# hao1635/FoundDiff

Measured on AMD Instinct MI355X. Metric: denoised CT slices/sec (512x512, 50 DDIM steps), higher is better.
Workload: dtype bf16; last 1 step(s): resolution levels 0-1 on the fp32s engine (fp32 storage, split-bf16 contractions: 3 bf16 MFMAs per product); 1 GPU; BASELINE configs[2]: 512x512 slice, 50-step DDIM, full FoundDiff UNet (dim 64, mults 1-2-4-8) + DA-CLIP RN50 cond, bf16; concurrent_sub_batches=2

## Files before the change

### founddiff_amd/csrc/fd_initconv.hip

```cpp
#include "fd_common.h"

namespace {

constexpr int IT = 16, IHY = IT + 6, IHX = IT + 8;

template <int NG>
__global__ __launch_bounds__(256, 2) void initconv7_kernel(const float *__restrict__ p0, const float *__restrict__ p1,
                                                          const float *__restrict__ p2, const bf16 *__restrict__ wk,
                                                          const float *__restrict__ bias, bf16 *__restrict__ out,
                                                          int H, int W) {
    __shared__ __attribute__((aligned(16))) uint2 sx[IHY * IHX];
    const int tid = threadIdx.x, lane = tid & 63, wave = tid >> 6;
    const int fr = lane & 15, fg = lane >> 4;
    const int tiles_x = W / IT;
    const int ty0 = (blockIdx.x / tiles_x) * IT, tx0 = (blockIdx.x % tiles_x) * IT;
    const int64_t img = blockIdx.y, plane = (int64_t)H * W;
    const int rperm = 8 * (fr >> 2) + (fr & 3);
    bf16x8 wa[NG][7], wb[NG][7];
#pragma unroll
    for (int g = 0; g < NG; ++g)
#pragma unroll
        for (int kh = 0; kh < 7; ++kh) {
            wa[g][kh] = *(const bf16x8 *)(wk + (int64_t)(32 * g + rperm) * 224 + kh * 32 + fg * 8);
            wb[g][kh] = *(const bf16x8 *)(wk + (int64_t)(32 * g + rperm + 4) * 224 + kh * 32 + fg * 8);
        }
    for (int i = tid; i < IHY * IHX; i += 256) {
        const int hy = i / IHX, hx = i - hy * IHX;
        const int y = ty0 + hy - 3, x = tx0 + hx - 3;
        float v0 = 0.f, v1 = 0.f, v2 = 0.f;
        if (y >= 0 && y < H && x >= 0 && x < W) {
            const int64_t o = img * plane + (int64_t)y * W + x;
            v0 = p0[o];
            if (p1) v1 = p1[o];
            if (p2) v2 = p2[o];
        }
        const bf16 b0 = (bf16)v0, b1 = (bf16)v1;
        uint2 wv;
        wv.x = (uint32_t)__builtin_bit_cast(uint16_t, b0) | ((uint32_t)__builtin_bit_cast(uint16_t, b1) << 16);
        if (p2) {
            const bf16 b2 = (bf16)v2;
            wv.y = (uint32_t)__builtin_bit_cast(uint16_t, b2);
        } else {
            const bf16 l0 = (bf16)(v0 - (float)b0), l1 = (bf16)(v1 - (float)b1);
            wv.y = (uint32_t)__builtin_bit_cast(uint16_t, l0) | ((uint32_t)__builtin_bit_cast(uint16_t, l1) << 16);
        }
        sx[i] = wv;
    }
    __syncthreads();
    float bs[NG][8];
#pragma unroll
    for (int g = 0; g < NG; ++g) {
        if (bias) load8(bias + 32 * g + 8 * fg, bs[g]);
        else {
#pragma unroll
            for (int e = 0; e < 8; ++e) bs[g][e] = 0.f;
        }
    }
    constexpr int CO = 32 * NG;
#pragma unroll 1
    for (int i = 0; i < 4; ++i) {
        const int ty = 4 * wave + i;
        f32x4 a0[NG], a1[NG];
#pragma unroll
        for (int g = 0; g < NG; ++g) { a0[g] = (f32x4){0.f, 0.f, 0.f, 0.f}; a1[g] = (f32x4){0.f, 0.f, 0.f, 0.f}; }
#pragma unroll
        for (int kh = 0; kh < 7; ++kh) {
            const uint2 *src = sx + (ty + kh) * IHX + fr + 2 * fg;
            const uint2 q0 = src[0], q1 = src[1];
            const u32x4 xv = {q0.x, q0.y, q1.x, q1.y};
            const bf16x8 xb = __builtin_bit_cast(bf16x8, xv);
#pragma unroll
            for (int g = 0; g < NG; ++g) {
                a0[g] = FD_MFMA16(wa[g][kh], xb, a0[g], 0, 0, 0);
                a1[g] = FD_MFMA16(wb[g][kh], xb, a1[g], 0, 0, 0);
            }
        }
        const int y = ty0 + ty, x = tx0 + fr;
        bf16 *op = out + ((img * H + y) * W + x) * CO + 8 * fg;
#pragma unroll
        for (int g = 0; g < NG; ++g) {
            float val[8];
#pragma unroll
            for (int e = 0; e < 4; ++e) { val[e] = a0[g][e] + bs[g][e]; val[4 + e] = a1[g][e] + bs[g][4 + e]; }
            store8(op + 32 * g, val);
        }
    }
}

template <int NG>
__global__ __launch_bounds__(256, 2) void initconv7_f32s_kernel(const float *__restrict__ p0, const float *__restrict__ p1,
                                                               const bf16 *__restrict__ wk, const bf16 *__restrict__ wl,
                                                               const float *__restrict__ bias, float *__restrict__ out,
                                                               int H, int W) {
    __shared__ __attribute__((aligned(16))) uint2 sx[IHY * IHX];
    const int tid = threadIdx.x, lane = tid & 63, wave = tid >> 6;
    const int fr = lane & 15, fg = lane >> 4;
    const int tiles_x = W / IT;
    const int ty0 = (blockIdx.x / tiles_x) * IT, tx0 = (blockIdx.x % tiles_x) * IT;
    const int64_t img = blockIdx.y, plane = (int64_t)H * W;
    const int rperm = 8 * (fr >> 2) + (fr & 3);
    for (int i = tid; i < IHY * IHX; i += 256) {
        const int hy = i / IHX, hx = i - hy * IHX;
        const int y = ty0 + hy - 3, x = tx0 + hx - 3;
        float v0 = 0.f, v1 = 0.f;
        if (y >= 0 && y < H && x >= 0 && x < W) {
            const int64_t o = img * plane + (int64_t)y * W + x;
            v0 = p0[o];
            v1 = p1[o];
        }
        const bf16 b0 = (bf16)v0, b1 = (bf16)v1;
        const bf16 l0 = (bf16)(v0 - (float)b0), l1 = (bf16)(v1 - (float)b1);
        uint2 wv;
        wv.x = (uint32_t)__builtin_bit_cast(uint16_t, b0) | ((uint32_t)__builtin_bit_cast(uint16_t, b1) << 16);
        wv.y = (uint32_t)__builtin_bit_cast(uint16_t, l0) | ((uint32_t)__builtin_bit_cast(uint16_t, l1) << 16);
        sx[i] = wv;
    }
    __syncthreads();
    constexpr int CO = 32 * NG;
#pragma unroll 1
    for (int g = 0; g < NG; ++g) {
        bf16x8 wa[7], wb[7], la[7], lb[7];
#pragma unroll
        for (int kh = 0; kh < 7; ++kh) {
            const int64_t oa = (int64_t)(32 * g + rperm) * 224 + kh * 32 + fg * 8, ob = oa + 4 * 224;
            wa[kh] = *(const bf16x8 *)(wk + oa);
            wb[kh] = *(const bf16x8 *)(wk + ob);
            la[kh] = *(const bf16x8 *)(wl + oa);
            lb[kh] = *(const bf16x8 *)(wl + ob);
        }
        float bs[8];
        if (bias) load8(bias + 32 * g + 8 * fg, bs);
        else {
#pragma unroll
            for (int e = 0; e < 8; ++e) bs[e] = 0.f;
        }
#pragma unroll 1
        for (int i = 0; i < 4; ++i) {
            const int ty = 4 * wave + i;
            f32x4 a0 = {0.f, 0.f, 0.f, 0.f}, a1 = {0.f, 0.f, 0.f, 0.f};
#pragma unroll
            for (int kh = 0; kh < 7; ++kh) {
                const uint2 *src = sx + (ty + kh) * IHX + fr + 2 * fg;
                const uint2 q0 = src[0], q1 = src[1];
                const u32x4 xv = {q0.x, q0.y, q1.x, q1.y};
                const bf16x8 xb = __builtin_bit_cast(bf16x8, xv);
                a0 = FD_MFMA16(la[kh], xb, a0, 0, 0, 0);
                a1 = FD_MFMA16(lb[kh], xb, a1, 0, 0, 0);
                a0 = FD_MFMA16(wa[kh], xb, a0, 0, 0, 0);
                a1 = FD_MFMA16(wb[kh], xb, a1, 0, 0, 0);
            }
            const int y = ty0 + ty, x = tx0 + fr;
            float *op = out + ((img * H + y) * W + x) * CO + 32 * g + 8 * fg;
            float val[8];
#pragma unroll
            for (int e = 0; e < 4; ++e) { val[e] = a0[e] + bs[e]; val[4 + e] = a1[e] + bs[4 + e]; }
            store8(op, val);
        }
    }
}

}

extern "C" int fd_init_conv7_f32s(const float *p0, const float *p1, const void *w_hi_packed, const void *w_lo_packed,
                                  const float *bias, void *out, int B, int H, int W, int Cout, void *stream) {
    FD_REQUIRE((Cout == 32 || Cout == 64) && H % IT == 0 && W % IT == 0, "fd_init_conv7_f32s: needs Cout in {32, 64}, H, W multiples "
               "of 16 (Cout=%d H=%d W=%d)", Cout, H, W);
    FD_REQUIRE(p0 && p1 && w_hi_packed && w_lo_packed && out, "fd_init_conv7_f32s: null pointer");
    FD_REQUIRE((((uintptr_t)bias | (uintptr_t)out | (uintptr_t)w_hi_packed | (uintptr_t)w_lo_packed) & 15) == 0, "fd_init_conv7_f32s: 16-byte alignment");
    dim3 grid((H / IT) * (W / IT), B), block(256);
    if (Cout == 64)
        hipLaunchKernelGGL(initconv7_f32s_kernel<2>, grid, block, 0, (hipStream_t)stream, p0, p1, (const bf16 *)w_hi_packed,
                           (const bf16 *)w_lo_packed, bias, (float *)out, H, W);
    else
        hipLaunchKernelGGL(initconv7_f32s_kernel<1>, grid, block, 0, (hipStream_t)stream, p0, p1, (const bf16 *)w_hi_packed,
                           (const bf16 *)w_lo_packed, bias, (float *)out, H, W);
    FD_LAUNCH_OK("fd_init_conv7_f32s");
    return FD_OK;
}

extern "C" int fd_init_conv7_ok(int dtype, int Cout, int H, int W) {
    return dtype == FD_BF16 && (Cout == 32 || Cout == 64) && H % IT == 0 && W % IT == 0;
}

extern "C" int fd_init_conv7(int dtype, const float *p0, const float *p1, const float *p2, const void *w_packed,
                             const float *bias, void *out, int B, int H, int W, int Cout, void *stream) {
    FD_REQUIRE(fd_init_conv7_ok(dtype, Cout, H, W), "fd_init_conv7: needs bf16, Cout in {32, 64}, H, W multiples of 16 "
               "(Cout=%d H=%d W=%d)", Cout, H, W);
    FD_REQUIRE(p0 && w_packed && out, "fd_init_conv7: null pointer");
    FD_REQUIRE(!bias || ((uintptr_t)bias & 15) == 0, "fd_init_conv7: bias must be 16-byte aligned");
    dim3 grid((H / IT) * (W / IT), B), block(256);
    if (Cout == 64)
        hipLaunchKernelGGL(initconv7_kernel<2>, grid, block, 0, (hipStream_t)stream, p0, p1, p2, (const bf16 *)w_packed, bias,
                           (bf16 *)out, H, W);
    else
        hipLaunchKernelGGL(initconv7_kernel<1>, grid, block, 0, (hipStream_t)stream, p0, p1, p2, (const bf16 *)w_packed, bias,
                           (bf16 *)out, H, W);
    FD_LAUNCH_OK("fd_init_conv7");
    return FD_OK;
}
```

### founddiff_amd/csrc/fd_scan.hip

```cpp
#include "fd_common.h"
#include <stdlib.h>

namespace {

struct ScanGeom {
    int B, H, W, D, N, R, CD;
    int H2, W2, L, CL, nch;
    const void *xw;
    float *xdbl_out;
    bool low_latency;
};

__device__ __forceinline__ void scan_pos(const ScanGeom &g, int k, int l, int &lrow, int &pix) {
    int h2, w2;
    if (k & 1) { w2 = l / g.H2; h2 = l - w2 * g.H2; }
    else { h2 = l / g.W2; w2 = l - h2 * g.W2; }
    lrow = h2 * g.W2 + w2;
    pix = (2 * h2 + (k & 1)) * g.W + 2 * w2 + (k >> 1);
}

template <typename T, int N, int R, bool FINAL, bool ODD, int CPL = 1>
__global__ __launch_bounds__(256, (N >= 32 ? 3 : (N >= 16 && R >= 16 ? 4 : (N >= 8 ? (CPL == 2 ? 4 : 5) : 1)))) void scan_chunk_kernel(const T *__restrict__ xc, const float *__restrict__ xdbl,
                                                        const float *__restrict__ dtw, const float *__restrict__ dtb,
                                                        const float *__restrict__ A, const float *__restrict__ Ds,
// ... 141 lines not shown
                    }
                }
            }
        }
    }
    if (FINAL || !g.xw)
    for (int idx = threadIdx.x; idx < (l1 - l0) * CD; idx += blockDim.x) {
        const int row = idx / CD, e = idx - row * CD;
        const int l = l0 + row;
        int h2, w2;
        if (odd) { w2 = l / g.H2; h2 = l - w2 * g.H2; }
        else { h2 = l / g.W2; w2 = l - h2 * g.W2; }
        float v = xb[(int64_t)(h2 * g.W2 + w2) * CD + e];
        if (LOG2U && FINAL && e >= R + N) v *= 0.6931471805599453f;
        sx[row * CDP + e] = v;
    }

    constexpr int NP = CPL == 2 ? N : N / 2, RP = CPL == 2 ? R : R / 2;
    f32x2 w[RP], a2[NP], h[NP];
    f32x2 bias2 = {0.f, 0.f}, Dd2 = {0.f, 0.f};
    float bias = 0.f, Dd = 0.f;
    const int64_t cbase = (((int64_t)bk * g.nch + chunk) * N) * g.D + d;
    if constexpr (CPL == 2) {
#pragma unroll
        for (int r = 0; r < R; ++r) w[r] = f32x2{dtw[(int64_t)kd * R + r], dtw[(int64_t)(kd + 1) * R + r]} * WS;
#pragma unroll
        for (int n = 0; n < N; ++n) a2[n] = f32x2{A[(int64_t)kd * N + n], A[(int64_t)(kd + 1) * N + n]} * AS;
        bias2 = f32x2{dtb[kd], dtb[kd + 1]} * WS;
        if (FINAL) Dd2 = f32x2{Ds[kd], Ds[kd + 1]};
#pragma unroll
        for (int n = 0; n < N; ++n) h[n] = FINAL ? *(const f32x2 *)&wsH[cbase + (int64_t)n * g.D] : f32x2{0.f, 0.f};
    } else {
#pragma unroll
        for (int r = 0; r < R / 2; ++r) w[r] = f32x2{dtw[(int64_t)kd * R + 2 * r], dtw[(int64_t)kd * R + 2 * r + 1]} * WS;
#pragma unroll
        for (int n = 0; n < N / 2; ++n)
            a2[n] = f32x2{A[(int64_t)kd * N + 2 * n], A[(int64_t)kd * N + 2 * n + 1]} * AS;
        bias = dtb[kd] * WS;
        Dd = FINAL ? Ds[kd] : 0.f;
        if (FINAL) {
#pragma unroll
            for (int n = 0; n < N / 2; ++n)
                h[n] = f32x2{wsH[cbase + (int64_t)(2 * n) * g.D], wsH[cbase + (int64_t)(2 * n + 1) * g.D]};
        } else {
#pragma unroll
            for (int n = 0; n < N / 2; ++n) h[n] = f32x2{0.f, 0.f};
        }
    }
    float sdt = 0.f;
    f32x2 sdt2 = {0.f, 0.f};
    const T *ub = xc + (int64_t)b * g.H * g.W * g.D;
    T *yb = FINAL ? y + (int64_t)b * g.H * g.W * g.D : nullptr;
    const int rowb = g.D * (int)sizeof(T);
    const int img_bytes = g.H * g.W * rowb;
    const __amdgpu_buffer_rsrc_t rs_u = __builtin_amdgcn_make_buffer_rsrc((void *)ub, 0, img_bytes, 0x00020000);
    const __amdgpu_buffer_rsrc_t rs_y = __builtin_amdgcn_make_buffer_rsrc((void *)(FINAL ? yb : (T *)ub), 0, img_bytes, 0x00020000);
    const int voff = d * (int)sizeof(T);
    auto ld_u = [&](int soff_) -> uint32_t {
        const int soff = __builtin_amdgcn_readfirstlane(soff_);
        if (ODD && soff < 0) return 0u;
        if constexpr (CPL == 2) return __builtin_amdgcn_raw_buffer_load_b32(rs_u, voff, soff, 0);
        else if constexpr (sizeof(T) == 2) return (uint32_t)__builtin_amdgcn_raw_buffer_load_b16(rs_u, voff, soff, 0);
        else return __builtin_amdgcn_raw_buffer_load_b32(rs_u, voff, soff, 0);
    };
    auto cvt_u = [&](uint32_t r) -> float {
        if constexpr (sizeof(T) == 2) return fd_h_lo(r);
        else return __builtin_bit_cast(float, r);
    };
    auto st_y = [&](int soff_, float v) {
        const int soff = __builtin_amdgcn_readfirstlane(soff_);
        if (ODD && soff < 0) return;
        if constexpr (sizeof(T) == 2) {
            const bf16 hv = fd_cvt_h(v);
            __builtin_amdgcn_raw_buffer_store_b16(__builtin_bit_cast(unsigned short, hv), rs_y, voff, soff, 0);
        } else {
            __builtin_amdgcn_raw_buffer_store_b32(__builtin_bit_cast(uint32_t, v), rs_y, voff, soff, 0);
        }
    };
    auto st_y2 = [&](int soff_, f32x2 v) {
        const int soff = __builtin_amdgcn_readfirstlane(soff_);
        if (ODD && soff < 0) return;
        typedef __attribute__((ext_vector_type(2))) bf16 bfx2;
        const bfx2 hv = {fd_cvt_h(v.x), fd_cvt_h(v.y)};
        __builtin_amdgcn_raw_buffer_store_b32(__builtin_bit_cast(uint32_t, hv), rs_y, voff, soff, 0);
    };
    const int NI = odd ? g.H2 : g.W2;
    const int s_i = odd ? 2 * g.W : 2, s_o = odd ? 2 : 2 * g.W;
    int ci = __builtin_amdgcn_readfirstlane(l0 % NI);
    int pixc = __builtin_amdgcn_readfirstlane(ph * g.W + pw + (l0 % NI) * s_i + (l0 / NI) * s_o);
    const int wrap_fix = s_o - NI * s_i;
    const int NO = odd ? g.W2 : g.H2;
    const bool padF = ODD && (odd ? ((g.H & 1) && ph) : ((g.W & 1) && pw));
    const bool padS = ODD && (odd ? ((g.W & 1) && pw) : ((g.H & 1) && ph));
    int co = __builtin_amdgcn_readfirstlane(l0 / NI);
    __syncthreads();

    constexpr int NXV = CPL == 2 ? ((FINAL ? CD : R + N) + 3) / 4 : 1;
    struct RowV { f32x4 v[NXV]; };
    auto ld_row = [&](int li) -> RowV {
        RowV q;
#pragma unroll
        for (int c = 0; c < NXV; ++c) q.v[c] = *(const f32x4 *)&sx[li * CDP + 4 * c];
        return q;
    };
    auto step = [&](const float *xr_lds, const RowV &rq, uint32_t uraw, int soff) {
        if constexpr (CPL == 2) {
            const auto xr = [&](int i) -> float { return rq.v[i >> 2][i & 3]; };
            const f32x2 u2 = {fd_h_lo(uraw), fd_h_hi(uraw)};
            f32x2 dv2 = bias2;
#pragma unroll
            for (int r = 0; r < R; ++r) dv2 = w[r] * xr(r) + dv2;
            f32x2 dt2;
            dt2.x = __builtin_amdgcn_logf(1.0f + __builtin_amdgcn_exp2f(fminf(dv2.x, 126.f)));
            dt2.y = __builtin_amdgcn_logf(1.0f + __builtin_amdgcn_exp2f(fminf(dv2.y, 126.f)));
            const f32x2 dtu2 = dt2 * u2;
            if (!FINAL) sdt2 += dt2;
            f32x2 acc2 = Dd2 * u2;
#pragma unroll
            for (int n = 0; n < N; ++n) {
                const f32x2 t = a2[n] * dt2;
                const f32x2 da = {__builtin_amdgcn_exp2f(t.x), __builtin_amdgcn_exp2f(t.y)};
                h[n] = da * h[n] + dtu2 * xr(R + n);
                if (FINAL) acc2 = h[n] * xr(R + N + n) + acc2;
            }
            if (FINAL) st_y2(soff, acc2);
        } else {
        const float u = cvt_u(uraw);
        const f32x2 *xr2 = (const f32x2 *)xr_lds;
        f32x2 dv2 = {bias, 0.f};
#pragma unroll
        for (int r = 0; r < R / 2; ++r) dv2 = w[r] * xr2[r] + dv2;
        const float dv = dv2.x + dv2.y;
        float dt;
        if constexpr (LOG2U) dt = __builtin_amdgcn_logf(1.0f + __builtin_amdgcn_exp2f(fminf(dv, 126.f)));
        else dt = fd_softplus_fast(dv);
        const float dtu = dt * u;
        if (!FINAL) sdt += dt;
        f32x2 acc2 = {0.f, 0.f};
#pragma unroll
        for (int n = 0; n < N / 2; ++n) {
            const f32x2 t = a2[n] * dt;
            const f32x2 da = {__builtin_amdgcn_exp2f(t.x), __builtin_amdgcn_exp2f(t.y)};
            h[n] = da * h[n] + xr2[R / 2 + n] * dtu;
            if (FINAL) acc2 = h[n] * xr2[R / 2 + N / 2 + n] + acc2;
        }
        if (FINAL) st_y(soff, acc2.x + acc2.y + Dd * u);
        }
    };
    auto advance = [&](int &soff) {
        soff = pixc * rowb;
        if (ODD && ((padF && ci == NI - 1) || (padS && co == NO - 1))) soff = -1;
        ++ci;
        const bool wrap = ci == NI;
        ci = wrap ? 0 : ci;
        if (ODD) co += wrap ? 1 : 0;
        pixc += s_i + (wrap ? wrap_fix : 0);
    };
    if constexpr (!FINAL && CPL == 2) {
        if (g.xw) {
            unsigned char *su = (unsigned char *)(sx + g.CL * CDP);
            const bf16 *Wk = (const bf16 *)g.xw + (int64_t)k * CD * g.D;
            const bf16 *ubx = (const bf16 *)xc + (int64_t)b * g.H * g.W * g.D;
            float *xo = g.xdbl_out + ((int64_t)k * g.B + b) * g.L * g.CD;
            constexpr int MB = (CD + 15) / 16, KSM = 4;
            const int fr = lane & 15, fg = lane >> 4;
            const int nblk = (l1 - l0 + 15) >> 4;
            struct BlkPos { int l, lrow; };
            auto bfetch = [&](int nb, BlkPos &q, bf16x8 (&bq)[KSM]) {
                const int l = l0 + nb * 16 + fr;
                int h2, w2;
                if (odd) { w2 = l / g.H2; h2 = l - w2 * g.H2; }
                else { h2 = l / g.W2; w2 = l - h2 * g.W2; }
                const int hh = 2 * h2 + ph, ww = 2 * w2 + pw;
                const bool inimg = l < l1 && hh < g.H && ww < g.W;
                const bf16 *px = ubx + ((int64_t)hh * g.W + ww) * g.D + 8 * fg;
                q.l = l;
                q.lrow = h2 * g.W2 + w2;
#pragma unroll
                for (int ks = 0; ks < KSM; ++ks) {
                    bq[ks] = (bf16x8){0, 0, 0, 0, 0, 0, 0, 0};
                    if (inimg) bq[ks] = *(const bf16x8 *)(px + 32 * ks);
                }
            };
            bf16x8 afr[MB][KSM];
#pragma unroll
            for (int mb = 0; mb < MB; ++mb) {
                const int e = mb * 16 + fr;
#pragma unroll
                for (int ks = 0; ks < KSM; ++ks) {
                    afr[mb][ks] = (bf16x8){0, 0, 0, 0, 0, 0, 0, 0};
                    if (e < CD) afr[mb][ks] = *(const bf16x8 *)(Wk + (int64_t)e * g.D + 32 * ks + 8 * fg);
                }
            }
            const int su_rd = ((lane >> 2) << 4) | ((lane & 3) << 2);
            auto ld_su = [&](int s_) -> uint32_t { return *(const uint32_t *)(su + s_ * 256 + (su_rd ^ ((s_ & 15) << 4))); };
            BlkPos cur, nxt;
            bf16x8 bcur[KSM], bnxt[KSM];
            bfetch(0, cur, bcur);
            for (int nb = 0; nb < nblk; ++nb) {
                const bool more = nb + 1 < nblk;
                if (more) bfetch(nb + 1, nxt, bnxt);
#pragma unroll
                for (int mb = 0; mb < MB; ++mb) {
                    f32x4 acc = {0.f, 0.f, 0.f, 0.f};
#pragma unroll
                    for (int ks = 0; ks < KSM; ++ks) acc = FD_MFMA16(afr[mb][ks], bcur[ks], acc, 0, 0, 0);
                    const int e0 = mb * 16 + 4 * fg;
                    if (cur.l < l1 && e0 < CD) {
                        *(f32x4 *)&sx[(nb * 16 + fr) * CDP + e0] = acc;
                        *(f32x4 *)&xo[(int64_t)cur.lrow * CD + e0] = acc;
                    }
                }
#pragma unroll
                for (int ks = 0; ks < KSM; ++ks) *(bf16x8 *)(su + fr * 256 + (((ks * 4 + fg) ^ fr) << 4)) = bcur[ks];
                const int ns = min(16, l1 - l0 - nb * 16);
                if (ns == 16) {
                    RowV r0 = ld_row(nb * 16);
                    uint32_t u0 = ld_su(0);
#pragma unroll
                    for (int st = 0; st < 16; ++st) {
                        RowV r1 = r0;
                        uint32_t u1 = u0;
                        if (st + 1 < 16) { r1 = ld_row(nb * 16 + st + 1); u1 = ld_su(st + 1); }
                        __builtin_amdgcn_sched_barrier(0);
                        step(nullptr, r0, u0, 0);
                        r0 = r1;
                        u0 = u1;
                    }
                } else {
                    for (int st = 0; st < ns; ++st) step(nullptr, ld_row(nb * 16 + st), ld_su(st), 0);
                }
                if (more) {
                    cur = nxt;
#pragma unroll
                    for (int ks = 0; ks < KSM; ++ks) bcur[ks] = bnxt[ks];
                }
            }
#pragma unroll
            for (int n = 0; n < N; ++n) *(f32x2 *)&wsH[cbase + (int64_t)n * g.D] = h[n];
            *(f32x2 *)&wsP[((int64_t)bk * g.nch + chunk) * g.D + d] = sdt2;
            return;
        }
    }
    constexpr int U = (N >= 16) ? 8 : 16;
    int l = l0;
    const int ngroups = (l1 - l0) / U;
    int pixA[U], pixB[U];
    uint32_t uA[U], uB[U];
    auto fetch = [&](int (&pix)[U], uint32_t (&u)[U]) {
#pragma unroll
        for (int s = 0; s < U; ++s) advance(pix[s]);
#pragma unroll
        for (int s = 0; s < U; ++s) u[s] = ld_u(pix[s]);
    };
    auto run = [&](const int (&pix)[U], const uint32_t (&u)[U]) {
        if constexpr (CPL == 2) {
            RowV r0 = ld_row(l - l0);
#pragma unroll
            for (int s = 0; s < U; ++s) {
                RowV r1 = r0;
                if (s + 1 < U) r1 = ld_row(l - l0 + s + 1);
                __builtin_amdgcn_sched_barrier(0);
                step(nullptr, r0, u[s], pix[s]);
                r0 = r1;
            }
        } else {
            const RowV none = {};
#pragma unroll
            for (int s = 0; s < U; ++s) step(sx + (l - l0 + s) * CDP, none, u[s], pix[s]);
        }
        l += U;
    };
    if (ngroups > 0) fetch(pixA, uA);
    for (int gi = 0; gi < ngroups; gi += 2) {
        if (gi + 1 < ngroups) fetch(pixB, uB);
        run(pixA, uA);
        if (gi + 1 < ngroups) {
            if (gi + 2 < ngroups) fetch(pixA, uA);
            run(pixB, uB);
        }
    }
    for (; l < l1; ++l) {
        int soff;
        advance(soff);
        step(sx + (l - l0) * CDP, ld_row(l - l0), ld_u(soff), soff);
    }
    if (!FINAL) {
        if constexpr (CPL == 2) {
#pragma unroll
            for (int n = 0; n < N; ++n) *(f32x2 *)&wsH[cbase + (int64_t)n * g.D] = h[n];
            *(f32x2 *)&wsP[((int64_t)bk * g.nch + chunk) * g.D + d] = sdt2;
        } else {
#pragma unroll
            for (int n = 0; n < N / 2; ++n) {
                wsH[cbase + (int64_t)(2 * n) * g.D] = h[n].x;
                wsH[cbase + (int64_t)(2 * n + 1) * g.D] = h[n].y;
            }
            wsP[((int64_t)bk * g.nch + chunk) * g.D + d] = sdt;
        }
    }
}

constexpr int SEG = 16;
template <int PER>
__global__ __launch_bounds__(64 * SEG) void scan_carry_kernel(float *__restrict__ wsH, const float *__restrict__ wsS,
                                                             const float *__restrict__ A, float a_scale, int nch,
                                                             int N, int D) {
    __shared__ float sP[SEG][64], sH[SEG][64];
    const int lane = threadIdx.x & 63;
    const int seg = __builtin_amdgcn_readfirstlane(threadIdx.x >> 6);
    const int dblocks = D / 64;
    const int db = blockIdx.x % dblocks, n = (blockIdx.x / dblocks) % N, bk = blockIdx.x / (dblocks * N);
    const int d = db * 64 + lane;
    const int per = (nch + SEG - 1) / SEG;
    const int c0 = seg * per, c1 = min(c0 + per, nch);
    const int64_t base = ((int64_t)bk * nch * N + n) * D + d;
    const int64_t cs = (int64_t)N * D;
    const float *sd = wsS + (int64_t)bk * nch * D + d;
    const float a2 = A[((int64_t)(bk & 3) * D + d) * N + n] * a_scale;
    if constexpr (PER == 0) {
        float P = 1.f, Hh = 0.f;
        for (int c = c0; c < c1; ++c) {
            const float p = __builtin_amdgcn_exp2f(a2 * sd[(int64_t)c * D]), hh = wsH[base + c * cs];
            Hh = p * Hh + hh;
            P = p * P;
        }
        sP[seg][lane] = P;
        sH[seg][lane] = Hh;
        __syncthreads();
        float carry = 0.f;
        for (int s = 0; s < seg; ++s) carry = sP[s][lane] * carry + sH[s][lane];
        for (int c = c0; c < c1; ++c) {
            const float p = __builtin_amdgcn_exp2f(a2 * sd[(int64_t)c * D]), hh = wsH[base + c * cs];
            wsH[base + c * cs] = carry;
            carry = p * carry + hh;
        }
        return;
    }
    constexpr int PR = PER > 0 ? PER : 1;
    float pv[PR], hv[PR];
    const float *ps = sd + (int64_t)c0 * D;
    float *ph = wsH + base + c0 * cs;
#pragma unroll
    for (int u = 0; u < PER; ++u) {
        pv[u] = 0.f;
        hv[u] = 0.f;
        if (c0 + u < c1) {
            pv[u] = *ps;
            hv[u] = *ph;
        }
        ps += D;
        ph += cs;
    }
    float P = 1.f, Hh = 0.f;
#pragma unroll
    for (int u = 0; u < PER; ++u) {
        if (c0 + u < c1) {
            pv[u] = __builtin_amdgcn_exp2f(a2 * pv[u]);
            Hh = pv[u] * Hh + hv[u];
            P = pv[u] * P;
        }
    }
    sP[seg][lane] = P;
    sH[seg][lane] = Hh;
    __syncthreads();
    float carry = 0.f;
    for (int s = 0; s < seg; ++s) carry = sP[s][lane] * carry + sH[s][lane];
    ph = wsH + base + c0 * cs;
#pragma unroll
    for (int u = 0; u < PER; ++u) {
        if (c0 + u < c1) {
            *ph = carry;
            carry = pv[u] * carry + hv[u];
        }
        ph += cs;
    }
}

constexpr int SEQ_LPC = 4, SEQ_SP = 32, SEQ_MAXL = 1024;

__device__ __forceinline__ float quad_sum(float v) {
    v += __builtin_bit_cast(float, __builtin_amdgcn_update_dpp(0, __builtin_bit_cast(int, v), 0xB1, 0xF, 0xF, true));
    v += __builtin_bit_cast(float, __builtin_amdgcn_update_dpp(0, __builtin_bit_cast(int, v), 0x4E, 0xF, 0xF, true));
    return v;
}

template <typename T, int N, int R, bool ODD>
__global__ __launch_bounds__(256) void scan_seq_kernel(const T *__restrict__ xc, const float *__restrict__ xdbl,
                                                      const float *__restrict__ dtw, const float *__restrict__ dtb,
                                                      const float *__restrict__ A, const float *__restrict__ Ds,
                                                      T *__restrict__ y, const ScanGeom g) {
    constexpr int LPC = SEQ_LPC, NS = N / LPC, RS = R / LPC, SP = SEQ_SP;
    constexpr int CD = R + 2 * N, CD4 = CD / 4;
    static_assert(NS % 2 == 0 && RS % 2 == 0 && CD % 4 == 0 && (R + N) % 4 == 0, "scan_seq_kernel: slice shapes");
    constexpr bool LOG2U = sizeof(T) == 2;
    constexpr float WS = LOG2U ? 1.4426950408889634f : 1.f;
    constexpr float AS = LOG2U ? 1.f : 1.4426950408889634f;
    constexpr int CDS = CD + 4;
    __shared__ __attribute__((aligned(16))) float sx[2][SP * CDS];
    const int tid = threadIdx.x, lane = tid & 63;
    const int wave = __builtin_amdgcn_readfirstlane(tid >> 6);
    const int sub = lane & 3;
    const int bk = blockIdx.y, b = bk >> 2, k = bk & 3;
    const int d = blockIdx.x * 64 + wave * 16 + (lane >> 2);
    const int kd = k * g.D + d;
    const int odd = k & 1, ph = k & 1, pw = k >> 1;
    const float *xb = xdbl + ((int64_t)k * g.B + b) * g.L * CD;

    f32x2 w[R / 2], a2[NS / 2], h[NS / 2];
#pragma unroll
    for (int r = 0; r < R / 2; ++r)
        w[r] = f32x2{dtw[(int64_t)kd * R + 2 * r], dtw[(int64_t)kd * R + 2 * r + 1]} * WS;
#pragma unroll
    for (int n = 0; n < NS / 2; ++n) {
        a2[n] = f32x2{A[(int64_t)kd * N + sub * NS + 2 * n], A[(int64_t)kd * N + sub * NS + 2 * n + 1]} * AS;
        h[n] = f32x2{0.f, 0.f};
    }
    const float bias = dtb[kd] * WS;
    const float Dd = Ds[kd];

    const T *ub = xc + (int64_t)b * g.H * g.W * g.D;
    T *yb = y + (int64_t)b * g.H * g.W * g.D;
    const int rowb = g.D * (int)sizeof(T);
    const int img_bytes = g.H * g.W * rowb;
    const __amdgpu_buffer_rsrc_t rs_u = __builtin_amdgcn_make_buffer_rsrc((void *)ub, 0, img_bytes, 0x00020000);
    const __amdgpu_buffer_rsrc_t rs_y = __builtin_amdgcn_make_buffer_rsrc((void *)yb, 0, img_bytes, 0x00020000);
    const int voff = d * (int)sizeof(T);
    auto ld_u = [&](int soff_) -> uint32_t {
        const int soff = __builtin_amdgcn_readfirstlane(soff_);
        if (ODD && soff < 0) return 0u;
        if constexpr (sizeof(T) == 2) return (uint32_t)__builtin_amdgcn_raw_buffer_load_b16(rs_u, voff, soff, 0);
        else return __builtin_amdgcn_raw_buffer_load_b32(rs_u, voff, soff, 0);
    };
    auto cvt_u = [&](uint32_t r) -> float {
        if constexpr (sizeof(T) == 2) return fd_h_lo(r);
        else return __builtin_bit_cast(float, r);
    };
    auto st_y = [&](int soff_, float v) {
        const int soff = __builtin_amdgcn_readfirstlane(soff_);
        if (ODD && soff < 0) return;
        if constexpr (sizeof(T) == 2) {
            const bf16 hv = fd_cvt_h(v);
            __builtin_amdgcn_raw_buffer_store_b16(__builtin_bit_cast(unsigned short, hv), rs_y, voff, soff, 0);
        } else {
            __builtin_amdgcn_raw_buffer_store_b32(__builtin_bit_cast(uint32_t, v), rs_y, voff, soff, 0);
        }
    };
    const int NI = odd ? g.H2 : g.W2;
    const int s_i = odd ? 2 * g.W : 2, s_o = odd ? 2 : 2 * g.W;
    int ci = 0, co = 0;
    int pixc = __builtin_amdgcn_readfirstlane(ph * g.W + pw);
    const int wrap_fix = s_o - NI * s_i;
    const int NO = odd ? g.W2 : g.H2;
    const bool padF = ODD && (odd ? ((g.H & 1) && ph) : ((g.W & 1) && pw));
    const bool padS = ODD && (odd ? ((g.W & 1) && pw) : ((g.H & 1) && ph));
    auto advance = [&](int &soff) {
        soff = pixc * rowb;
        if (ODD && ((padF && ci == NI - 1) || (padS && co == NO - 1))) soff = -1;
        ++ci;
        const bool wrap = ci == NI;
        ci = wrap ? 0 : ci;
        if (ODD) co += wrap ? 1 : 0;
        pixc += s_i + (wrap ? wrap_fix : 0);
    };

    constexpr int NLD = (SP * CD4 + 255) / 256;
    f32x4 stg[NLD];
    auto load_rows = [&](int st) {
#pragma unroll
        for (int j = 0; j < NLD; ++j) {
            const int idx = tid + j * 256;
            const int r = idx / CD4, e4 = idx - r * CD4;
            const int l = st * SP + r;
            stg[j] = (f32x4){0.f, 0.f, 0.f, 0.f};
            if (idx < SP * CD4 && l < g.L) {
                int h2, w2;
                if (odd) { w2 = l / g.H2; h2 = l - w2 * g.H2; }
                else { h2 = l / g.W2; w2 = l - h2 * g.W2; }
                f32x4 v = *(const f32x4 *)(xb + (int64_t)(h2 * g.W2 + w2) * CD + 4 * e4);
                if (LOG2U && 4 * e4 >= R + N) v = v * 0.6931471805599453f;
                stg[j] = v;
            }
        }
    };
    auto store_rows = [&](int buf) {
#pragma unroll
        for (int j = 0; j < NLD; ++j) {
            const int idx = tid + j * 256;
            if (idx < SP * CD4) *(f32x4 *)&sx[buf][(idx / CD4) * CDS + 4 * (idx % CD4)] = stg[j];
        }
    };
    auto lds_barrier = [&]() { asm volatile("s_waitcnt lgkmcnt(0)\n\ts_barrier" ::: "memory"); };

    struct RowRegs { f32x2 br[NS / 2], cr[NS / 2]; };
    auto load_row = [&](const float *xr, RowRegs &q) {
        const f32x2 *br2 = (const f32x2 *)(xr + R + sub * NS);
        const f32x2 *cr2 = (const f32x2 *)(xr + R + N + sub * NS);
#pragma unroll
        for (int n = 0; n < NS / 2; ++n) { q.br[n] = br2[n]; q.cr[n] = cr2[n]; }
    };
    auto dt_of_row = [&](const float *xr) -> float {
        const f32x2 *wr2 = (const f32x2 *)xr;
        f32x2 dv2 = {0.f, 0.f}, dv3 = {0.f, 0.f};
#pragma unroll
        for (int r = 0; r < R / 2; ++r) {
            if (r & 1) dv3 = w[r] * wr2[r] + dv3;
            else dv2 = w[r] * wr2[r] + dv2;
        }
        const float dv = ((dv2.x + dv3.x) + (dv2.y + dv3.y)) + bias;
        if constexpr (LOG2U) return __builtin_amdgcn_logf(1.0f + __builtin_amdgcn_exp2f(fminf(dv, 126.f)));
        else return fd_softplus_fast(dv);
    };
    struct PreOut { f32x2 da[NS / 2], bdu[NS / 2]; float du; };
    auto pre = [&](const RowRegs &q, uint32_t uraw, float dt, PreOut &o) {
        const float u = cvt_u(uraw);
        const float dtu = dt * u;
        o.du = Dd * u;
#pragma unroll
        for (int n = 0; n < NS / 2; ++n) {
            const f32x2 t = a2[n] * dt;
            o.da[n] = f32x2{__builtin_amdgcn_exp2f(t.x), __builtin_amdgcn_exp2f(t.y)};
            o.bdu[n] = q.br[n] * dtu;
        }
    };
    auto post = [&](const RowRegs &q, const PreOut &o, int soff) {
        f32x2 acc2 = {0.f, 0.f}, acc3 = {0.f, 0.f};
#pragma unroll
        for (int n = 0; n < NS / 2; ++n) {
            h[n] = o.da[n] * h[n] + o.bdu[n];
            if (n & 1) acc3 = h[n] * q.cr[n] + acc3;
            else acc2 = h[n] * q.cr[n] + acc2;
        }
        st_y(soff, quad_sum((acc2.x + acc3.x) + (acc2.y + acc3.y)) + o.du);
    };

    constexpr int U = 8;
    const int G = g.L / U;
    int pixA[U], pixB[U];
    uint32_t uA[U], uB[U];
    auto fetch = [&](int (&pix)[U], uint32_t (&u)[U]) {
#pragma unroll
        for (int s = 0; s < U; ++s) advance(pix[s]);
#pragma unroll
        for (int s = 0; s < U; ++s) u[s] = ld_u(pix[s]);
    };
    auto quad_bcast = [&](float v, int i) -> float {
        const int x = __builtin_bit_cast(int, v);
        int r;
        if (i == 0) r = __builtin_amdgcn_update_dpp(0, x, 0x00, 0xF, 0xF, true);
        else if (i == 1) r = __builtin_amdgcn_update_dpp(0, x, 0x55, 0xF, 0xF, true);
        else if (i == 2) r = __builtin_amdgcn_update_dpp(0, x, 0xAA, 0xF, 0xF, true);
        else r = __builtin_amdgcn_update_dpp(0, x, 0xFF, 0xF, 0xF, true);
        return __builtin_bit_cast(float, r);
    };
    auto run = [&](int gi, const int (&pix)[U], const uint32_t (&u)[U]) {
        const float *rows = &sx[(gi >> 2) & 1][((gi & 3) * U) * CDS];
        RowRegs q[3];
        PreOut o[2];
        float dtq[U / 4];
        load_row(rows, q[0]);
        load_row(rows + CDS, q[1]);
        dtq[0] = dt_of_row(rows + sub * CDS);
        pre(q[0], u[0], quad_bcast(dtq[0], 0), o[0]);
#pragma unroll
        for (int s = 0; s < U; ++s) {
            if (s + 2 < U) load_row(rows + (s + 2) * CDS, q[(s + 2) % 3]);
            __builtin_amdgcn_sched_barrier(0);
            if ((s & 3) == 0 && s + 4 < U) dtq[s / 4 + 1] = dt_of_row(rows + (s + 4 + sub) * CDS);
            if (s + 1 < U) pre(q[(s + 1) % 3], u[s + 1], quad_bcast(dtq[(s + 1) / 4], (s + 1) & 3), o[(s + 1) & 1]);
            post(q[s % 3], o[s & 1], pix[s]);
        }
    };
    load_rows(0);
    store_rows(0);
    if (SP < g.L) load_rows(1);
    if (G > 0) fetch(pixA, uA);
    lds_barrier();
    for (int gi = 0; gi < G; gi += 2) {
        if (gi + 1 < G) fetch(pixB, uB);
        run(gi, pixA, uA);
        if (gi + 1 < G) {
            if (gi + 2 < G) fetch(pixA, uA);
            run(gi + 1, pixB, uB);
            if ((gi & 3) == 2) {
                const int st = gi >> 2;
                if ((st + 1) * SP < g.L) store_rows((st + 1) & 1);
                lds_barrier();
                if ((st + 2) * SP < g.L) load_rows(st + 2);
            }
        }
    }
    for (int l = G * U; l < g.L; ++l) {
        int soff;
        advance(soff);
        RowRegs q;
        PreOut o;
        const float *xr = &sx[(l / SP) & 1][(l % SP) * CDS];
        load_row(xr, q);
        pre(q, ld_u(soff), dt_of_row(xr), o);
        post(q, o, soff);
    }
}

bool scan_seq_ok(int H, int W, int D, int N, int R) {
    const bool off = fd_dev(FD_DEV_SCAN_NO_SEQ);
    if (off) return false;
    const int L = ((H + 1) / 2) * ((W + 1) / 2);
    return L <= SEQ_MAXL && N >= 16 && N % (2 * SEQ_LPC) == 0 && R % (2 * SEQ_LPC) == 0 && D % 64 == 0;
}

template <typename T, int N, int R, bool ODD>
void launch_scan_seq(const T *xc, const float *xdbl, const float *dtw, const float *dtb, const float *A,
                     const float *Ds, T *y, const ScanGeom &g, hipStream_t s) {
    if constexpr (N >= 16 && N % (2 * SEQ_LPC) == 0 && R % (2 * SEQ_LPC) == 0) {
        dim3 grid(g.D / 64, g.B * 4), block(256);
        hipLaunchKernelGGL((scan_seq_kernel<T, N, R, ODD>), grid, block, 0, s, xc, xdbl, dtw, dtb, A, Ds, y, g);
    }
}

__global__ __launch_bounds__(256) void scan_zero_kernel(float *__restrict__ p, int64_t n) {
    const int64_t i = (int64_t)blockIdx.x * 256 + threadIdx.x;
    if (i < n) p[i] = 0.f;
}
// ... 203 lines not shown
```

Baseline: 13.73 slices/s.

## Make init conv persistent with double-buffered halo prefetch; hold scan carry in registers

The 7x7 init conv becomes a persistent grid sized to two workgroups per CU. Each block loops over tiles, prefetching the next tile's halo into registers while the current tile's MFMAs run from a double-buffered LDS tile, and loads its weights only once. Separately, the scan carry kernel gets a register-held path for up to 32 chunks per segment: it loads the chunk values once, computes exp2 once, and reuses them in the second pass instead of re-reading global memory. These add register pressure and static code, and the persistent grid may balance load worse across CUs.

```diff
diff --git a/founddiff_amd/csrc/fd_initconv.hip b/founddiff_amd/csrc/fd_initconv.hip
--- a/founddiff_amd/csrc/fd_initconv.hip
+++ b/founddiff_amd/csrc/fd_initconv.hip
@@ -4,17 +4,19 @@
 
 constexpr int IT = 16, IHY = IT + 6, IHX = IT + 8;
 
+constexpr int IHN = (IHY * IHX + 255) / 256;
+constexpr int IWG_PER_CU = 2;
+
 template <int NG>
-__global__ __launch_bounds__(256, 2) void initconv7_kernel(const float *__restrict__ p0, const float *__restrict__ p1,
-                                                          const float *__restrict__ p2, const bf16 *__restrict__ wk,
-                                                          const float *__restrict__ bias, bf16 *__restrict__ out,
-                                                          int H, int W) {
-    __shared__ __attribute__((aligned(16))) uint2 sx[IHY * IHX];
+__global__ __launch_bounds__(256, IWG_PER_CU) void initconv7_kernel(const float *__restrict__ p0, const float *__restrict__ p1,
+                                                                   const float *__restrict__ p2, const bf16 *__restrict__ wk,
+                                                                   const float *__restrict__ bias, bf16 *__restrict__ out,
+                                                                   int H, int W, int ntiles) {
+    __shared__ __attribute__((aligned(16))) uint2 sx[2][IHY * IHX];
     const int tid = threadIdx.x, lane = tid & 63, wave = tid >> 6;
     const int fr = lane & 15, fg = lane >> 4;
-    const int tiles_x = W / IT;
-    const int ty0 = (blockIdx.x / tiles_x) * IT, tx0 = (blockIdx.x % tiles_x) * IT;
-    const int64_t img = blockIdx.y, plane = (int64_t)H * W;
+    const int tiles_x = W / IT, tiles_img = (H / IT) * tiles_x;
+    const int64_t plane = (int64_t)H * W;
     const int rperm = 8 * (fr >> 2) + (fr & 3);
     bf16x8 wa[NG][7], wb[NG][7];
 #pragma unroll
@@ -24,29 +26,6 @@
             wa[g][kh] = *(const bf16x8 *)(wk + (int64_t)(32 * g + rperm) * 224 + kh * 32 + fg * 8);
             wb[g][kh] = *(const bf16x8 *)(wk + (int64_t)(32 * g + rperm + 4) * 224 + kh * 32 + fg * 8);
         }
-    for (int i = tid; i < IHY * IHX; i += 256) {
-        const int hy = i / IHX, hx = i - hy * IHX;
-        const int y = ty0 + hy - 3, x = tx0 + hx - 3;
-        float v0 = 0.f, v1 = 0.f, v2 = 0.f;
-        if (y >= 0 && y < H && x >= 0 && x < W) {
-            const int64_t o = img * plane + (int64_t)y * W + x;
-            v0 = p0[o];
-            if (p1) v1 = p1[o];
-            if (p2) v2 = p2[o];
-        }
-        const bf16 b0 = (bf16)v0, b1 = (bf16)v1;
-        uint2 wv;
-        wv.x = (uint32_t)__builtin_bit_cast(uint16_t, b0) | ((uint32_t)__builtin_bit_cast(uint16_t, b1) << 16);
-        if (p2) {
-            const bf16 b2 = (bf16)v2;
-            wv.y = (uint32_t)__builtin_bit_cast(uint16_t, b2);
-        } else {
-            const bf16 l0 = (bf16)(v0 - (float)b0), l1 = (bf16)(v1 - (float)b1);
-            wv.y = (uint32_t)__builtin_bit_cast(uint16_t, l0) | ((uint32_t)__builtin_bit_cast(uint16_t, l1) << 16);
-        }
-        sx[i] = wv;
-    }
-    __syncthreads();
     float bs[NG][8];
 #pragma unroll
     for (int g = 0; g < NG; ++g) {
@@ -56,35 +35,107 @@
             for (int e = 0; e < 8; ++e) bs[g][e] = 0.f;
         }
     }
+    int hy[IHN], hx[IHN];
+#pragma unroll
+    for (int k = 0; k < IHN; ++k) {
+        const int i = tid + 256 * k;
+        hy[k] = i / IHX - 3;
+        hx[k] = i % IHX - 3;
+    }
+    float v0[IHN], v1[IHN], v2[IHN];
+    auto tile_at = [&](int t, int64_t &img, int &ty0, int &tx0) {
+        const int b = t / tiles_img, r = t - b * tiles_img;
+        img = b;
+        ty0 = (r / tiles_x) * IT;
+        tx0 = (r % tiles_x) * IT;
+    };
+    auto fetch = [&](int t) {
+        int64_t img;
+        int ty0, tx0;
+        tile_at(t, img, ty0, tx0);
+#pragma unroll
+        for (int k = 0; k < IHN; ++k) {
+            v0[k] = 0.f; v1[k] = 0.f; v2[k] = 0.f;
+            const int y = ty0 + hy[k], x = tx0 + hx[k];
+            if (tid + 256 * k < IHY * IHX && y >= 0 && y < H && x >= 0 && x < W) {
+                const int64_t o = img * plane + (int64_t)y * W + x;
+                v0[k] = p0[o];
+                if (p1) v1[k] = p1[o];
+                if (p2) v2[k] = p2[o];
+            }
+        }
+    };
+    auto stash = [&](uint2 *dst) {
+#pragma unroll
+        for (int k = 0; k < IHN; ++k) {
+            if (tid + 256 * k >= IHY * IHX) continue;
+            const bf16 b0 = (bf16)v0[k], b1 = (bf16)v1[k];
+            uint2 wv;
+            wv.x = (uint32_t)__builtin_bit_cast(uint16_t, b0) | ((uint32_t)__builtin_bit_cast(uint16_t, b1) << 16);
+            if (p2) {
+                const bf16 b2 = (bf16)v2[k];
+                wv.y = (uint32_t)__builtin_bit_cast(uint16_t, b2);
+            } else {
+                const bf16 l0 = (bf16)(v0[k] - (float)b0), l1 = (bf16)(v1[k] - (float)b1);
+                wv.y = (uint32_t)__builtin_bit_cast(uint16_t, l0) | ((uint32_t)__builtin_bit_cast(uint16_t, l1) << 16);
+            }
+            dst[tid + 256 * k] = wv;
+        }
+    };
     constexpr int CO = 32 * NG;
-#pragma unroll 1
-    for (int i = 0; i < 4; ++i) {
-        const int ty = 4 * wave + i;
-        f32x4 a0[NG], a1[NG];
-#pragma unroll
-        for (int g = 0; g < NG; ++g) { a0[g] = (f32x4){0.f, 0.f, 0.f, 0.f}; a1[g] = (f32x4){0.f, 0.f, 0.f, 0.f}; }
-#pragma unroll
-        for (int kh = 0; kh < 7; ++kh) {
-            const uint2 *src = sx + (ty + kh) * IHX + fr + 2 * fg;
-            const uint2 q0 = src[0], q1 = src[1];
-            const u32x4 xv = {q0.x, q0.y, q1.x, q1.y};
-            const bf16x8 xb = __builtin_bit_cast(bf16x8, xv);
+    int t = blockIdx.x, buf = 0;
+    if (t < ntiles) fetch(t);
+#pragma unroll 1
+    for (; t < ntiles; t += gridDim.x, buf ^= 1) {
+        const uint2 *sxb = sx[buf];
+        stash(sx[buf]);
+        __syncthreads();
+        if (t + (int)gridDim.x < ntiles) fetch(t + gridDim.x);
+        int64_t img;
+        int ty0, tx0;
+        tile_at(t, img, ty0, tx0);
+#pragma unroll 1
+        for (int i = 0; i < 4; ++i) {
+            const int ty = 4 * wave + i;
+            f32x4 a0[NG], a1[NG];
+#pragma unroll
+            for (int g = 0; g < NG; ++g) { a0[g] = (f32x4){0.f, 0.f, 0.f, 0.f}; a1[g] = (f32x4){0.f, 0.f, 0.f, 0.f}; }
+#pragma unroll
+            for (int kh = 0; kh < 7; ++kh) {
+                const uint2 *src = sxb + (ty + kh) * IHX + fr + 2 * fg;
+                const uint2 q0 = src[0], q1 = src[1];
+                const u32x4 xv = {q0.x, q0.y, q1.x, q1.y};
+                const bf16x8 xb = __builtin_bit_cast(bf16x8, xv);
+#pragma unroll
+                for (int g = 0; g < NG; ++g) {
+                    a0[g] = FD_MFMA16(wa[g][kh], xb, a0[g], 0, 0, 0);
+                    a1[g] = FD_MFMA16(wb[g][kh], xb, a1[g], 0, 0, 0);
+                }
+            }
+            const int y = ty0 + ty, x = tx0 + fr;
+            bf16 *op = out + ((img * H + y) * W + x) * CO + 8 * fg;
 #pragma unroll
             for (int g = 0; g < NG; ++g) {
-                a0[g] = FD_MFMA16(wa[g][kh], xb, a0[g], 0, 0, 0);
-                a1[g] = FD_MFMA16(wb[g][kh], xb, a1[g], 0, 0, 0);
-            }
-        }
-        const int y = ty0 + ty, x = tx0 + fr;
-        bf16 *op = out + ((img * H + y) * W + x) * CO + 8 * fg;
-#pragma unroll
-        for (int g = 0; g < NG; ++g) {
-            float val[8];
-#pragma unroll
-            for (int e = 0; e < 4; ++e) { val[e] = a0[g][e] + bs[g][e]; val[4 + e] = a1[g][e] + bs[g][4 + e]; }
-            store8(op + 32 * g, val);
-        }
-    }
+                float val[8];
+#pragma unroll
+                for (int e = 0; e < 4; ++e) { val[e] = a0[g][e] + bs[g][e]; val[4 + e] = a1[g][e] + bs[g][4 + e]; }
+                store8(op + 32 * g, val);
+            }
+        }
+    }
+}
+
+int initconv7_grid(int64_t ntiles) {
+    static int cus[64];
+    int dev = 0;
+    if (hipGetDevice(&dev) != hipSuccess || dev < 0 || dev >= 64) dev = 0;
+    if (cus[dev] == 0) {
+        int n = 0;
+        if (hipDeviceGetAttribute(&n, hipDeviceAttributeMultiprocessorCount, dev) != hipSuccess || n <= 0) n = 256;
+        cus[dev] = n;
+    }
+    const int64_t wg = (int64_t)IWG_PER_CU * cus[dev];
+    return (int)(ntiles < wg ? ntiles : wg);
 }
 
 template <int NG>
@@ -188,13 +239,15 @@
                "(Cout=%d H=%d W=%d)", Cout, H, W);
     FD_REQUIRE(p0 && w_packed && out, "fd_init_conv7: null pointer");
     FD_REQUIRE(!bias || ((uintptr_t)bias & 15) == 0, "fd_init_conv7: bias must be 16-byte aligned");
-    dim3 grid((H / IT) * (W / IT), B), block(256);
+    const int64_t ntiles = (int64_t)B * (H / IT) * (W / IT);
+    FD_REQUIRE(B >= 1 && ntiles < (1ll << 31), "fd_init_conv7: B x tiles must fit 31 bits (B=%d H=%d W=%d)", B, H, W);
+    dim3 grid(initconv7_grid(ntiles)), block(256);
     if (Cout == 64)
         hipLaunchKernelGGL(initconv7_kernel<2>, grid, block, 0, (hipStream_t)stream, p0, p1, p2, (const bf16 *)w_packed, bias,
-                           (bf16 *)out, H, W);
+                           (bf16 *)out, H, W, (int)ntiles);
     else
         hipLaunchKernelGGL(initconv7_kernel<1>, grid, block, 0, (hipStream_t)stream, p0, p1, p2, (const bf16 *)w_packed, bias,
-                           (bf16 *)out, H, W);
+                           (bf16 *)out, H, W, (int)ntiles);
     FD_LAUNCH_OK("fd_init_conv7");
     return FD_OK;
 }
diff --git a/founddiff_amd/csrc/fd_scan.hip b/founddiff_amd/csrc/fd_scan.hip
--- a/founddiff_amd/csrc/fd_scan.hip
+++ b/founddiff_amd/csrc/fd_scan.hip
@@ -467,6 +467,38 @@
 }
 
 constexpr int SEG = 16;
+template <int PR>
+__device__ __forceinline__ void scan_carry_held(float *__restrict__ hu0, const float *__restrict__ su0, int64_t cs, int D, int nch,
+                                                int c0, int c1, float a2, int seg, unsigned lane, float (&sP)[SEG][64],
+                                                float (&sH)[SEG][64]) {
+    float pv[PR], hv[PR];
+#pragma unroll
+    for (int u = 0; u < PR; ++u) {
+        const int c = min(c0 + u, nch - 1);
+        pv[u] = (su0 + (int64_t)c * D)[lane];
+        hv[u] = (hu0 + c * cs)[lane];
+    }
+    float P = 1.f, Hh = 0.f;
+#pragma unroll
+    for (int u = 0; u < PR; ++u) {
+        const bool in = c0 + u < c1;
+        pv[u] = __builtin_amdgcn_exp2f(a2 * pv[u]);
+        const float h1 = pv[u] * Hh + hv[u], p1 = pv[u] * P;
+        Hh = in ? h1 : Hh;
+        P = in ? p1 : P;
+    }
+    sP[seg][lane] = P;
+    sH[seg][lane] = Hh;
+    __syncthreads();
+    float carry = 0.f;
+    for (int s = 0; s < seg; ++s) carry = sP[s][lane] * carry + sH[s][lane];
+#pragma unroll
+    for (int u = 0; u < PR; ++u) {
+        if (c0 + u < c1) (hu0 + (c0 + u) * cs)[lane] = carry;
+        carry = pv[u] * carry + hv[u];
+    }
+}
+
 template <int PER>
 __global__ __launch_bounds__(64 * SEG) void scan_carry_kernel(float *__restrict__ wsH, const float *__restrict__ wsS,
                                                              const float *__restrict__ A, float a_scale, int nch,
@@ -484,6 +516,13 @@
     const float *sd = wsS + (int64_t)bk * nch * D + d;
     const float a2 = A[((int64_t)(bk & 3) * D + d) * N + n] * a_scale;
     if constexpr (PER == 0) {
+        if (per <= 32) {
+            float *hu0 = wsH + ((int64_t)bk * nch * N + n) * D + db * 64;
+            const float *su0 = wsS + (int64_t)bk * nch * D + db * 64;
+            if (per <= 16) scan_carry_held<16>(hu0, su0, cs, D, nch, c0, c1, a2, seg, (unsigned)lane, sP, sH);
+            else scan_carry_held<32>(hu0, su0, cs, D, nch, c0, c1, a2, seg, (unsigned)lane, sP, sH);
+            return;
+        }
         float P = 1.f, Hh = 0.f;
         for (int c = c0; c < c1; ++c) {
             const float p = __builtin_amdgcn_exp2f(a2 * sd[(int64_t)c * D]), hh = wsH[base + c * cs];
```

Result: no change. 13.78 slices/s, median of 6 (+0.3%).
